# NeptuneHub/AudioMuse-AI

Hardware: NVIDIA H100
Metric: tracks_per_sec_analysed_10s_48khz (higher is better)
Workload: dtype bf16

## Files before the change

### audiomuse-ai_b200/csrc/fused_block.cu

```cuda
#include "fused_block.cuh"

#include <type_traits>

#include "gemm_wgmma.cuh"
#include "tma_pipeline.cuh"

namespace am {
namespace fused {

using namespace ptx;

constexpr int kTile = 8;
constexpr int kChunk = 64;
constexpr int kMaxCout = 256;
constexpr int kMaxStages = 4;
constexpr size_t kSmemMax = 232448;
constexpr uint32_t kConsumerBar = 1;
constexpr int kParamRows = 9 + 1 + 1;
constexpr uint32_t kDwBytes = kParamRows * kChunk * 4;
using Ring = pipe::Ring<kMaxStages>;

__host__ __device__ constexpr int halo(int S) { return (kTile - 1) * S + 3; }
__host__ __device__ constexpr int halo_px(int S) { return halo(S) * halo(S); }
__host__ __device__ constexpr int halo_rows(int S) { return (halo_px(S) + 63) / 64 * 64; }

constexpr uint32_t round1k(uint32_t v) { return (v + 1023u) & ~1023u; }

__device__ __forceinline__ int e_off(int p, int g) { return p * 64 + ((g ^ (p & 7)) << 3); }

__device__ __forceinline__ uint32_t sw128(uint32_t row, uint32_t chunk) {
  return (row << 7) + (((chunk ^ row) & 7u) << 4);
}

struct Layout {
  uint32_t stage, w2, dw;
  uint32_t xs, a2, e, bars, extra;
  int stages;
  size_t smem;
};

static Layout layout(int S, bool has_expand, int cin_p, int cout_p, int stages) {
  const uint32_t hr = (uint32_t)halo_rows(S), hpx = (uint32_t)halo_px(S);
  const uint32_t kbx = has_expand ? (uint32_t)((cin_p + 63) / 64) : 0u;
  const uint32_t n2 = (uint32_t)((cout_p + 63) / 64 * 64);
  Layout l;
  l.w2 = has_expand ? kbx * kChunk * 128 : round1k(hpx * 128);
  l.dw = l.w2 + n2 * 128;
  l.stage = round1k(l.dw + kDwBytes);
  l.xs = 0;
  l.a2 = l.xs + kbx * hr * 128;
  l.e = l.a2 + kTile * kTile * 128;
  l.bars = l.e + (has_expand ? hpx * 128 : 0u);
  l.extra = l.bars + 2 * sizeof(uint64_t);
  l.stages = stages;
  l.smem = Ring::smem_bytes(l.stage, stages, l.extra);
  return l;
}

struct Args {
  const __nv_bfloat16* X;
  const float* params;
  const float* b2;
  __nv_bfloat16* Y;
  int H, W, Ho, Wo, tiles_y, tiles_x, num_tiles;
  int cin_p, cmid_p, cout_p, residual;
  Layout l;
};

enum Phase { kRingWait, kHaloWait, kExpandMma, kExpandEpi, kDepthwise, kProjectMma, kBarrier, kEpilogue, kIssue, kNumPhases };
#ifdef AM_FUSED_PHASES
static const char* const kPhaseNames[kNumPhases] = {"ring_wait", "halo_wait", "expand_mma", "expand_epi", "depthwise",
                                                     "project_mma", "barrier", "epilogue", "issue"};
__device__ unsigned long long g_phase_cycles[3][kNumPhases];
__device__ __forceinline__ long long clock_now() {
  long long v;
  asm volatile("mov.u64 %0, %%clock64;" : "=l"(v));
  return v;
}
struct PhaseClock {
  uint32_t acc[kNumPhases];
  long long t;
  __device__ __forceinline__ PhaseClock() : acc{}, t(clock_now()) {}
  __device__ __forceinline__ void lap(Phase p) {
    const long long n = clock_now();
    acc[p] += (uint32_t)(n - t);
    t = n;
  }
  __device__ __forceinline__ void flush(int wg) {
    for (int p = 0; p < kNumPhases; ++p) atomicAdd(&g_phase_cycles[wg][p], (unsigned long long)acc[p]);
  }
};
#else
struct PhaseClock {
  __device__ __forceinline__ void lap(Phase) {}
  __device__ __forceinline__ void flush(int) {}
};
#endif

template <int S, bool kExpand>
__global__ void __launch_bounds__(pipe::kThreads, 1)
fused_block_kernel(const __grid_constant__ CUtensorMap map_x, const __grid_constant__ CUtensorMap map_w1,
                   const __grid_constant__ CUtensorMap map_w2, const Args a) {
  extern __shared__ __align__(1024) uint8_t smem_raw[];
  constexpr int HALO = halo(S), HPX = halo_px(S), HR = halo_rows(S);
  Ring ring(smem_raw, a.l.stage, a.l.stages, a.l.extra);
  uint8_t* own = ring.extra();
  uint8_t* xs = own + a.l.xs;
  uint8_t* a2 = own + a.l.a2;
  uint64_t* xs_full = reinterpret_cast<uint64_t*>(own + a.l.bars);
  uint64_t* xs_empty = xs_full + 1;

  const int per_img = a.tiles_y * a.tiles_x;
  const int kbx = (a.cin_p + 63) / 64;
  const int n2_blocks = (a.cout_p + 63) / 64;

  if (threadIdx.x == 0) {
    prefetch_tensormap(&map_x);
    if (kExpand) prefetch_tensormap(&map_w1);
    prefetch_tensormap(&map_w2);
    mbar_init(xs_full, 1);
    mbar_init(xs_empty, pipe::kConsumerThreads);
    ring.init();
  }
  __syncthreads();

  if (threadIdx.x < 128) {
    regs_producer();
    if (threadIdx.x < 32 && elect_one_sync()) {
      PhaseClock clk;
      uint32_t xs_phase = 0;
      for (int tile = blockIdx.x; tile < a.num_tiles; tile += gridDim.x) {
        const int b = tile / per_img, ty = (tile % per_img) / a.tiles_x, tx = tile % a.tiles_x;
        const int gy0 = ty * kTile * S - 1, gx0 = tx * kTile * S - 1;
        if (kExpand) {
          clk.lap(kIssue);
          mbar_wait(xs_empty, xs_phase ^ 1);
          clk.lap(kHaloWait);
          mbar_expect_tx(xs_full, (uint32_t)(kbx * HPX * 128));
          for (int kb = 0; kb < kbx; ++kb) tma_load_4d(xs + kb * HR * 128, &map_x, xs_full, kb * 64, gx0, gy0, b);
          xs_phase ^= 1;
        }
        for (int c0 = 0; c0 < a.cmid_p; c0 += kChunk) {
          const uint32_t tx_bytes = (kExpand ? (uint32_t)kbx * kChunk * 128 : (uint32_t)HPX * 128) +
                                    (uint32_t)n2_blocks * 64 * 128 + kDwBytes;
          clk.lap(kIssue);
          const Ring::Slot s = ring.acquire(tx_bytes);
          clk.lap(kRingWait);
          if (kExpand) {
            for (int kb = 0; kb < kbx; ++kb) tma_load_2d(s.smem + kb * kChunk * 128, &map_w1, s.bar, kb * 64, c0);
          } else {
            tma_load_4d(s.smem, &map_x, s.bar, c0, gx0, gy0, b);
          }
          tma_load_2d(s.smem + a.l.w2, &map_w2, s.bar, c0, 0);
          bulk_load(s.smem + a.l.dw, a.params + (int64_t)c0 * kParamRows, kDwBytes, s.bar);
        }
      }
      clk.lap(kIssue);
      clk.flush(0);
    }
    return;
  }
  regs_consumer();
  const int ct = threadIdx.x - 128;
  const int wg = __shfl_sync(0xffffffffu, ct >> 7, 0), wt = ct & 127;
  const int warp = wt >> 5, lane = wt & 31, quad = lane & 3;
  __nv_bfloat16* e_own = reinterpret_cast<__nv_bfloat16*>(own + a.l.e);
  const int nchunks = (a.cmid_p + kChunk - 1) / kChunk;
  const bool ahead = a.l.stages > 1;

  constexpr int kEN0 = ((HPX + 7) / 8 + 1) / 2 * 8;
  constexpr int kEN1 = (HPX + 7) / 8 * 8 - kEN0;
  const int half = a.cout_p / 2;

  float acc1[kEN0 / 2];
  float acc2[kMaxCout / 4];
#pragma unroll
  for (int i = 0; i < kEN0 / 2; ++i) acc1[i] = 0.f;
#pragma unroll
  for (int i = 0; i < kMaxCout / 4; ++i) acc2[i] = 0.f;

  auto expand_issue = [&](const uint8_t* stage) {
    const uint32_t w1 = smem_u32(stage), px = smem_u32(xs) + (uint32_t)(wg * kEN0 * 128);
    auto issue = [&](auto width) {
      for (int kb = 0; kb < kbx; ++kb) {
        const uint64_t da = make_smem_desc(w1 + (uint32_t)(kb * kChunk * 128));
        const uint64_t db = make_smem_desc(px + (uint32_t)(kb * HR * 128));
        const int ksteps = min(4, (a.cin_p - kb * 64) / 16);
        for (int ks = 0; ks < ksteps; ++ks)
          wgmma_into<decltype(width)::value>(acc1, da + (uint64_t)(ks * 2), db + (uint64_t)(ks * 2),
                                             (kb | ks) ? 1u : 0u);
      }
    };
    wgmma_fence();
    if (wg == 0) issue(std::integral_constant<int, kEN0>{});
    else issue(std::integral_constant<int, kEN1>{});
    wgmma_commit();
  };
  auto inside_mask = [&](int gy0, int gx0) {
    int p0 = wg * kEN0 + 2 * quad;
    asm volatile("" : "+r"(p0));
    uint64_t m = 0;
#pragma unroll
    for (int j = 0; j < kEN0 / 8; ++j)
#pragma unroll
      for (int k = 0; k < 2; ++k) {
        const int p = p0 + 8 * j + k;
        const int gy = gy0 + p / HALO, gx = gx0 + p % HALO;
        if (gy >= 0 && gy < a.H && gx >= 0 && gx < a.W) m |= 1ull << (2 * j + k);
      }
    return m;
  };
  auto expand_epilogue = [&](const uint8_t* stage, int nch, uint64_t inside) {
    reg_fence(acc1);
    const float* b1 = reinterpret_cast<const float*>(stage + a.l.dw) + 10 * kChunk;
    const int r = 16 * warp + (lane >> 2);
    const float bias[2] = {b1[r], b1[r + 8]};
    const uint32_t keep[2] = {r < nch ? ~0u : 0u, r + 8 < nch ? ~0u : 0u};
    auto pack = [&](int j, int h) {
      const uint32_t bits = (uint32_t)(inside >> (2 * j));
      const uint32_t mask = ((bits & 1u) * 0xffffu | (bits & 2u) * 0x7fff8000u) & keep[h];
      const __nv_bfloat162 v = __floats2bfloat162_rn(relu6f(acc1[4 * j + 2 * h] + bias[h]),
                                                     relu6f(acc1[4 * j + 2 * h + 1] + bias[h]));
      return *reinterpret_cast<const uint32_t*>(&v) & mask;
    };
    auto store = [&](auto wgc) {
      constexpr int P0 = decltype(wgc)::value * kEN0;
      constexpr int NG = (decltype(wgc)::value ? kEN1 : kEN0) / 8;
      constexpr int NFULL = (HPX - P0) / 8 < NG ? (HPX - P0) / 8 : NG;
      const int mi = lane >> 3;
      const uint32_t e_base = smem_u32(e_own);
#pragma unroll
      for (int j = 0; j + 1 < NFULL; j += 2) {
        const int p = P0 + 8 * (j + (mi >> 1)) + (lane & 7);
        stmatrix_x4_trans(e_base + 2 * e_off(p, 2 * warp + (mi & 1)), pack(j, 0), pack(j, 1), pack(j + 1, 0),
                          pack(j + 1, 1));
      }
      if (NFULL % 2) {
        const int p = P0 + 8 * (NFULL - 1) + (lane & 7);
        stmatrix_x2_trans(e_base + 2 * e_off(p, 2 * warp + (mi & 1)), pack(NFULL - 1, 0), pack(NFULL - 1, 1));
      }
#pragma unroll
      for (int j = NFULL; j < NG; ++j)
#pragma unroll
        for (int h = 0; h < 2; ++h) {
          const uint32_t v = pack(j, h);
#pragma unroll
          for (int k = 0; k < 2; ++k) {
            const int p = P0 + 8 * j + 2 * quad + k;
            if (p < HPX)
              reinterpret_cast<uint16_t*>(e_own)[e_off(p, 2 * warp + h) + (lane >> 2)] = (uint16_t)(v >> (16 * k));
          }
        }
    };
    if (wg == 0) store(std::integral_constant<int, 0>{});
    else store(std::integral_constant<int, 1>{});
  };

  PhaseClock clk;
  uint32_t xs_phase = 0;
  for (int tile = blockIdx.x; tile < a.num_tiles; tile += gridDim.x) {
    const int b = tile / per_img, ty = (tile % per_img) / a.tiles_x, tx = tile % a.tiles_x;
    const int oy0 = ty * kTile, ox0 = tx * kTile;
    const int gy0 = oy0 * S - 1, gx0 = ox0 * S - 1;
    const uint64_t inside = kExpand ? inside_mask(gy0, gx0) : 0;
    if (kExpand) {
      mbar_wait(xs_full, xs_phase);
      xs_phase ^= 1;
      clk.lap(kHaloWait);
      const uint8_t* s0 = ring.wait_ptr();
      clk.lap(kRingWait);
      expand_issue(s0);
      wgmma_wait<0>();
      clk.lap(kExpandMma);
      expand_epilogue(s0, min(kChunk, a.cmid_p), inside);
      if (nchunks == 1) mbar_arrive(xs_empty);
      clk.lap(kExpandEpi);
    }

    for (int c = 0; c < nchunks; ++c) {
      const int c0 = c * kChunk, nch = min(kChunk, a.cmid_p - c0);
      const bool next = kExpand && c + 1 < nchunks;
      uint8_t* sp = ring.wait_ptr();
      clk.lap(kRingWait);
      const float* dwp = reinterpret_cast<const float*>(sp + a.l.dw);
      const __nv_bfloat16* e = kExpand ? e_own : reinterpret_cast<const __nv_bfloat16*>(sp);
      named_bar_sync(kConsumerBar, pipe::kConsumerThreads);
      clk.lap(kBarrier);
      const uint8_t* sn = nullptr;
      if (next && ahead) {
        sn = ring.wait_ahead_ptr();
        clk.lap(kRingWait);
        expand_issue(sn);
        clk.lap(kExpandMma);
      }

      {
        const int ox = ct >> 5, cp = lane, g = cp >> 2;
        uint32_t out[kTile] = {};
        if (2 * cp < nch) {
          float2 w[9];
#pragma unroll
          for (int t = 0; t < 9; ++t) w[t] = *reinterpret_cast<const float2*>(dwp + t * kChunk + 2 * cp);
          const float2 bias = *reinterpret_cast<const float2*>(dwp + 9 * kChunk + 2 * cp);
          float2 acc[kTile];
#pragma unroll
          for (int oy = 0; oy < kTile; ++oy) acc[oy] = bias;
          const __nv_bfloat16* col[8];
#pragma unroll
          for (int k = 0; k < 8; ++k) col[k] = e + ox * S * 64 + ((g ^ ((ox * S + k) & 7)) << 3) + 2 * (cp & 3);
#pragma unroll
          for (int iy = 0; iy < HALO; ++iy) {
            float2 v[3];
#pragma unroll
            for (int dx = 0; dx < 3; ++dx) {
              const int d = iy * HALO + dx;
              v[dx] = __bfloat1622float2(*reinterpret_cast<const __nv_bfloat162*>(col[d & 7] + d * 64));
            }
#pragma unroll
            for (int dy = 0; dy < 3; ++dy) {
              if (iy < dy || (iy - dy) % S != 0 || (iy - dy) / S >= kTile) continue;
              const int oy = (iy - dy) / S;
#pragma unroll
              for (int dx = 0; dx < 3; ++dx) {
                acc[oy].x = fmaf(v[dx].x, w[dy * 3 + dx].x, acc[oy].x);
                acc[oy].y = fmaf(v[dx].y, w[dy * 3 + dx].y, acc[oy].y);
              }
            }
          }
#pragma unroll
          for (int oy = 0; oy < kTile; ++oy) {
            const __nv_bfloat162 o = __floats2bfloat162_rn(relu6f(acc[oy].x), relu6f(acc[oy].y));
            out[oy] = *reinterpret_cast<const uint32_t*>(&o);
          }
        }
        uint8_t* arow = a2 + sw128(ox, g) + 4 * (cp & 3);
#pragma unroll
        for (int oy = 0; oy < kTile; ++oy) *reinterpret_cast<uint32_t*>(arow + oy * kTile * 128) = out[oy];
      }
      fence_proxy_async();
      clk.lap(kDepthwise);
      named_bar_sync(kConsumerBar, pipe::kConsumerThreads);
      clk.lap(kBarrier);

      wgmma_fence();
      {
        const uint64_t da = make_smem_desc(smem_u32(a2));
        const uint64_t db = make_smem_desc(smem_u32(sp) + a.l.w2 + (uint32_t)(wg * half * 128));
        auto project = [&](auto width) {
          for (int ks = 0; ks < nch / 16; ++ks)
            wgmma_into<decltype(width)::value>(acc2, da + (uint64_t)(ks * 2), db + (uint64_t)(ks * 2),
                                               (c0 | ks) ? 1u : 0u);
        };
        switch (half) {
          case 8: project(std::integral_constant<int, 8>{}); break;
          case 16: project(std::integral_constant<int, 16>{}); break;
          case 24: project(std::integral_constant<int, 24>{}); break;
          case 32: project(std::integral_constant<int, 32>{}); break;
          case 40: project(std::integral_constant<int, 40>{}); break;
          case 48: project(std::integral_constant<int, 48>{}); break;
          case 56: project(std::integral_constant<int, 56>{}); break;
          case 64: project(std::integral_constant<int, 64>{}); break;
          case 72: project(std::integral_constant<int, 72>{}); break;
          case 80: project(std::integral_constant<int, 80>{}); break;
          case 88: project(std::integral_constant<int, 88>{}); break;
          case 96: project(std::integral_constant<int, 96>{}); break;
          case 104: project(std::integral_constant<int, 104>{}); break;
          case 112: project(std::integral_constant<int, 112>{}); break;
          case 120: project(std::integral_constant<int, 120>{}); break;
          case 128: project(std::integral_constant<int, 128>{}); break;
        }
      }
      wgmma_commit();
      clk.lap(kProjectMma);

      if (next && !ahead) {
        wgmma_wait<0>();
        ring.release();
        sn = ring.wait_ptr();
        clk.lap(kRingWait);
        expand_issue(sn);
      }
      wgmma_wait<0>();
      reg_fence(acc2);
      if (!next || ahead) ring.release();
      clk.lap(kProjectMma);
      if (next) {
        expand_epilogue(sn, min(kChunk, a.cmid_p - c0 - kChunk), inside);
        if (c + 2 == nchunks) mbar_arrive(xs_empty);
        clk.lap(kExpandEpi);
      }
    }

#pragma unroll
    for (int h = 0; h < 2; ++h) {
      const int px = warp * 16 + (lane >> 2) + 8 * h;
      const int oy = oy0 + (px >> 3), ox = ox0 + (px & 7);
      if (oy >= a.Ho || ox >= a.Wo) continue;
      const int64_t pix = ((int64_t)b * a.Ho + oy) * a.Wo + ox;
#pragma unroll
      for (int j = 0; j < kMaxCout / 16; ++j) {
        if (8 * j >= half) break;
        const int n = wg * half + 8 * j + 2 * quad;
        float f0 = acc2[4 * j + 2 * h] + __ldg(&a.b2[n]);
        float f1 = acc2[4 * j + 2 * h + 1] + __ldg(&a.b2[n + 1]);
        if (a.residual) {
          const float2 r = __bfloat1622float2(*reinterpret_cast<const __nv_bfloat162*>(a.X + pix * a.cin_p + n));
          f0 += r.x;
          f1 += r.y;
        }
        *reinterpret_cast<__nv_bfloat162*>(a.Y + pix * a.cout_p + n) = __floats2bfloat162_rn(f0, f1);
      }
    }
    clk.lap(kEpilogue);
  }
  if (wt == 0) clk.flush(1 + wg);
}

static bool fits(const BlockDesc& d) {
  const size_t hr = (size_t)halo_rows(d.stride);
  const size_t kbx = d.has_expand ? (size_t)((d.cin_p + 63) / 64) : 0;
  const size_t n2 = (size_t)((d.cout_p + 63) / 64 * 64);
  const size_t set = kbx * hr * 128 + kbx * kChunk * 128 + n2 * 128 + 64 * 128 + hr * 128;
  return set + 1024 <= kSmemMax;
}

bool plan(const BlockDesc& d, Plan* out) {
  if (d.stride != 1 && d.stride != 2) return false;
  if (d.cout_p > kMaxCout || d.cout_p % 16 || d.cmid_p % 16 || d.cin_p % 16) return false;
  if (!d.has_expand && d.cin_p != d.cmid_p) return false;
  if (d.residual && (d.stride != 1 || d.cin_p != d.cout_p)) return false;
  if (!fits(d)) return false;
  Layout l = layout(d.stride, d.has_expand != 0, d.cin_p, d.cout_p, kMaxStages);
  for (int s = kMaxStages - 1; s >= 1 && l.smem > kSmemMax; --s) l = layout(d.stride, d.has_expand != 0, d.cin_p, d.cout_p, s);
  out->stages = l.stages;
  out->smem_bytes = l.smem;
  return out->smem_bytes <= kSmemMax;
}

template <int S, bool kExpand>
static int launch(const CUtensorMap& mx, const CUtensorMap& m1, const CUtensorMap& m2, const Args& a, size_t smem,
                  cudaStream_t st) {
  AM_TRY((allow_dynamic_smem<fused_block_kernel<S, kExpand>>(kSmemMax)));
  const int grid = std::max(1, std::min(a.num_tiles, sm_count()));
#ifdef AM_FUSED_PHASES
  void* counters = nullptr;
  AM_CUDA(cudaGetSymbolAddress(&counters, g_phase_cycles));
  AM_CUDA(cudaMemsetAsync(counters, 0, sizeof(g_phase_cycles), st));
#endif
  AM_LAUNCH((fused_block_kernel<S, kExpand>), grid, pipe::kThreads, smem, st, mx, m1, m2, a);
#ifdef AM_FUSED_PHASES
  unsigned long long c[3][kNumPhases];
  AM_CUDA(cudaStreamSynchronize(st));
  AM_CUDA(cudaMemcpyFromSymbol(c, g_phase_cycles, sizeof(c)));
  std::fprintf(stderr, "fused_phases H=%d W=%d cin=%d cmid=%d cout=%d S=%d stages=%d grid=%d tiles=%d", a.H, a.W,
               a.cin_p, a.cmid_p, a.cout_p, S, a.l.stages, grid, a.num_tiles);
  for (int w = 0; w < 3; ++w)
    for (int p = 0; p < kNumPhases; ++p) std::fprintf(stderr, " wg%d.%s=%llu", w, kPhaseNames[p], c[w][p]);
  std::fprintf(stderr, "\n");
#endif
  return AM_OK;
}

std::vector<float> pack_params(const std::vector<float>& wd, const std::vector<float>& bd, const std::vector<float>* b1,
                               int c_p) {
  const int chunks = (c_p + kChunk - 1) / kChunk;
  std::vector<float> out((size_t)chunks * kParamRows * kChunk, 0.f);
  for (int c = 0; c < c_p; ++c) {
    float* q = &out[((size_t)(c / kChunk) * kParamRows) * kChunk + c % kChunk];
    for (int t = 0; t < 9; ++t) q[t * kChunk] = wd[(size_t)t * c_p + c];
    q[9 * kChunk] = bd[c];
    if (b1) q[10 * kChunk] = (*b1)[c];
  }
  return out;
}

int run(const BlockDesc& d, const Plan& p, const __nv_bfloat16* X, const __nv_bfloat16* W1, const float* params,
        const __nv_bfloat16* W2, const float* b2, __nv_bfloat16* Y, int B, cudaStream_t st) {
  AM_CHECK(X && params && W2 && b2 && Y && (!d.has_expand || W1), "fused block: NULL operand");
  auto aligned16 = [](const void* q) { return (reinterpret_cast<uintptr_t>(q) & 15) == 0; };
  AM_CHECK(aligned16(X) && aligned16(W2) && aligned16(params) && (!d.has_expand || aligned16(W1)),
           "fused block: operands must be 16-byte aligned (TMA)");
  Args a{};
  a.X = X;
  a.params = params;
  a.b2 = b2;
  a.Y = Y;
  a.H = d.H;
  a.W = d.W;
  a.Ho = (d.H - 1) / d.stride + 1;
  a.Wo = (d.W - 1) / d.stride + 1;
  a.tiles_y = (a.Ho + kTile - 1) / kTile;
  a.tiles_x = (a.Wo + kTile - 1) / kTile;
  const int64_t tiles = (int64_t)B * a.tiles_y * a.tiles_x;
  AM_CHECK(tiles < ((int64_t)1 << 31), "fused block: %lld tiles is too many for one launch", (long long)tiles);
  a.num_tiles = (int)tiles;
  a.cin_p = d.cin_p;
  a.cmid_p = d.cmid_p;
  a.cout_p = d.cout_p;
  a.residual = d.residual;
  const Layout l = layout(d.stride, d.has_expand != 0, d.cin_p, d.cout_p, p.stages);
  AM_CHECK(l.smem == p.smem_bytes, "fused block: plan does not match the block");
  a.l = l;

  CUtensorMap mx, m1, m2;
  const int hl = halo(d.stride);
  AM_TRY(gemm::encode_map_nhwc_bf16(&mx, X, B, d.H, d.W, d.cin_p, hl, hl, true));
  AM_TRY(gemm::encode_map_bf16(&m2, W2, d.cmid_p, d.cout_p, d.cmid_p, (d.cout_p + 63) / 64 * 64));
  if (d.has_expand) AM_TRY(gemm::encode_map_bf16(&m1, W1, d.cin_p, d.cmid_p, d.cin_p, kChunk));
  else m1 = m2;
  if (d.stride == 1) return d.has_expand ? launch<1, true>(mx, m1, m2, a, l.smem, st) : launch<1, false>(mx, m1, m2, a, l.smem, st);
  return d.has_expand ? launch<2, true>(mx, m1, m2, a, l.smem, st) : launch<2, false>(mx, m1, m2, a, l.smem, st);
}

}
}
```

### audiomuse-ai_b200/csrc/fused_block.cuh

```cuda
#pragma once

#include "common.cuh"

namespace am {
namespace fused {

struct BlockDesc {
  int H, W;
  int cin_p, cmid_p, cout_p;
  int stride;
  int has_expand;
  int residual;
};

struct Plan {
  size_t smem_bytes = 0;
  int stages = 1;
};

bool plan(const BlockDesc& d, Plan* out);

std::vector<float> pack_params(const std::vector<float>& wd, const std::vector<float>& bd, const std::vector<float>* b1,
                               int c_p);

int run(const BlockDesc& d, const Plan& p, const __nv_bfloat16* X, const __nv_bfloat16* W1, const float* params,
        const __nv_bfloat16* W2, const float* b2, __nv_bfloat16* Y, int B, cudaStream_t st);

}
}
```

### audiomuse-ai_b200/csrc/gemm.cu

```cuda
#include "gemm_wgmma.cuh"
#include "tma_pipeline.cuh"

#include <mutex>

namespace am {
namespace gemm {

using pipe::kChunkK;
using pipe::kThreads;

constexpr int kBlockM = 128;
constexpr int kStages = 4;
constexpr int kATileBytes = kBlockM * kChunkK * 2;
constexpr int kMaxBlockN = 256;
constexpr size_t kSmemMax = 232448;
using Ring = pipe::Ring<kStages>;

using namespace ptx;

struct KernelArgs {
  int64_t M, N;
  int K;
  int block_n;
  int tiles_m, tiles_n;
// ... 196 lines not shown
  }
  if (!args.d_is_f32 && wt == 0) bulk_wait_group<0>();
}

__global__ void gemm_simt_kernel(const __nv_bfloat16* __restrict__ A, int64_t M, int64_t lda,
                                 const __nv_bfloat16* __restrict__ B, int64_t N, int64_t ldb, int K,
                                 KernelArgs args) {
  const int64_t n = (int64_t)blockIdx.x * blockDim.x + threadIdx.x;
  const int64_t m = blockIdx.y;
  if (n >= N || m >= M) return;
  float acc = 0.f;
  for (int k = 0; k < K; ++k) acc = fmaf(__bfloat162float(A[m * lda + k]), __bfloat162float(B[n * ldb + k]), acc);
  float v = acc * args.alpha;
  if (args.bias) v += args.bias[n];
  if (args.col_sub) v -= args.col_sub[n];
  if (args.act == 1) v = relu6f(v);
  else if (args.act == 2) v = fmaxf(v, 0.f);
  else if (args.act == 3) v *= fminf(fmaxf(fmaf(v, 1.0f / 6.0f, 0.5f), 0.f), 1.f);
  if (args.d_is_f32) {
    reinterpret_cast<float*>(args.D)[m * args.ldd + n] = v;
  } else {
    if (args.residual) v += __bfloat162float(args.residual[m * args.ld_res + n]);
    reinterpret_cast<__nv_bfloat16*>(args.D)[m * args.ldd + n] = __float2bfloat16_rn(v);
  }
}

typedef CUresult (*EncodeTiledFn)(CUtensorMap*, CUtensorMapDataType, cuuint32_t, void*, const cuuint64_t*,
                                  const cuuint64_t*, const cuuint32_t*, const cuuint32_t*, CUtensorMapInterleave,
                                  CUtensorMapSwizzle, CUtensorMapL2promotion, CUtensorMapFloatOOBfill);

static EncodeTiledFn g_encode = nullptr;
static std::once_flag g_encode_once;

static EncodeTiledFn get_encode() {
  std::call_once(g_encode_once, [] {
    void* fn = nullptr;
    cudaDriverEntryPointQueryResult qres;
    cudaError_t e = cudaGetDriverEntryPoint("cuTensorMapEncodeTiled", &fn, cudaEnableDefault, &qres);
    if (e == cudaSuccess && qres == cudaDriverEntryPointSuccess) g_encode = reinterpret_cast<EncodeTiledFn>(fn);
    cudaGetLastError();
  });
  return g_encode;
}

bool available() { return ensure_init() == AM_OK && device_cc() == 90 && get_encode() != nullptr; }

int encode_map_bf16(void* map_out, const void* base, int64_t inner, int64_t rows, int64_t pitch_elems, int box_rows) {
  AM_CHECK(get_encode() != nullptr, "cuTensorMapEncodeTiled unavailable");
  const cuuint64_t dims[2] = {(cuuint64_t)inner, (cuuint64_t)rows};
  const cuuint64_t strides[1] = {(cuuint64_t)pitch_elems * 2};
  const cuuint32_t box[2] = {(cuuint32_t)kChunkK, (cuuint32_t)box_rows};
  const cuuint32_t estr[2] = {1, 1};
  CUresult r = get_encode()(reinterpret_cast<CUtensorMap*>(map_out), CU_TENSOR_MAP_DATA_TYPE_BFLOAT16, 2,
                            const_cast<void*>(base), dims, strides, box, estr, CU_TENSOR_MAP_INTERLEAVE_NONE,
                            CU_TENSOR_MAP_SWIZZLE_128B, CU_TENSOR_MAP_L2_PROMOTION_L2_256B,
                            CU_TENSOR_MAP_FLOAT_OOB_FILL_NONE);
  if (r != CUDA_SUCCESS) {
    set_error("cuTensorMapEncodeTiled failed (%d) inner=%lld rows=%lld pitch=%lld box_rows=%d", (int)r,
              (long long)inner, (long long)rows, (long long)pitch_elems, box_rows);
    return AM_ERR_CUDA;
  }
  return AM_OK;
}

int encode_map_nhwc_bf16(void* map_out, const void* base, int64_t n, int64_t h, int64_t w, int64_t c, int box_w,
                         int box_h, bool swizzle) {
  AM_CHECK(get_encode() != nullptr, "cuTensorMapEncodeTiled unavailable");
  const cuuint64_t dims[4] = {(cuuint64_t)c, (cuuint64_t)w, (cuuint64_t)h, (cuuint64_t)n};
  const cuuint64_t strides[3] = {(cuuint64_t)(c * 2), (cuuint64_t)(w * c * 2), (cuuint64_t)(h * w * c * 2)};
  const cuuint32_t box[4] = {(cuuint32_t)kChunkK, (cuuint32_t)box_w, (cuuint32_t)box_h, 1};
  const cuuint32_t estr[4] = {1, 1, 1, 1};
  CUresult r = get_encode()(reinterpret_cast<CUtensorMap*>(map_out), CU_TENSOR_MAP_DATA_TYPE_BFLOAT16, 4,
                            const_cast<void*>(base), dims, strides, box, estr, CU_TENSOR_MAP_INTERLEAVE_NONE,
                            swizzle ? CU_TENSOR_MAP_SWIZZLE_128B : CU_TENSOR_MAP_SWIZZLE_NONE,
                            CU_TENSOR_MAP_L2_PROMOTION_L2_256B, CU_TENSOR_MAP_FLOAT_OOB_FILL_NONE);
  if (r != CUDA_SUCCESS) {
    set_error("cuTensorMapEncodeTiled failed (%d) nhwc=[%lld, %lld, %lld, %lld] box=%dx%d", (int)r, (long long)n,
              (long long)h, (long long)w, (long long)c, box_w, box_h);
    return AM_ERR_CUDA;
  }
  return AM_OK;
}

static int encode_map_d(CUtensorMap* map_out, void* D, int64_t cols, int64_t rows, int64_t pitch_elems, int box_cols) {
  const cuuint64_t dims[2] = {(cuuint64_t)cols, (cuuint64_t)rows};
  const cuuint64_t strides[1] = {(cuuint64_t)pitch_elems * 2};
  const cuuint32_t box[2] = {(cuuint32_t)box_cols, 64};
  const cuuint32_t estr[2] = {1, 1};
  const int sw = box_cols == 64 ? 128 : tail_swizzle_bytes(box_cols);
  const CUtensorMapSwizzle swizzle = sw == 128  ? CU_TENSOR_MAP_SWIZZLE_128B
                                     : sw == 64 ? CU_TENSOR_MAP_SWIZZLE_64B
                                     : sw == 32 ? CU_TENSOR_MAP_SWIZZLE_32B
                                                : CU_TENSOR_MAP_SWIZZLE_NONE;
  CUresult r = get_encode()(map_out, CU_TENSOR_MAP_DATA_TYPE_BFLOAT16, 2, D, dims, strides, box, estr,
                            CU_TENSOR_MAP_INTERLEAVE_NONE, swizzle, CU_TENSOR_MAP_L2_PROMOTION_NONE,
                            CU_TENSOR_MAP_FLOAT_OOB_FILL_NONE);
  if (r != CUDA_SUCCESS) {
    set_error("cuTensorMapEncodeTiled failed (%d) for D: cols=%lld rows=%lld pitch=%lld box_cols=%d", (int)r,
              (long long)cols, (long long)rows, (long long)pitch_elems, box_cols);
    return AM_ERR_CUDA;
  }
  return AM_OK;
}

static bool gemm_has_n(int n) {
  return n == 16 || n == 32 || n == 48 || n == 64 || n == 80 || n == 96 || n == 112 || n == 128 || n == 144 ||
         n == 160 || n == 192 || n == 224 || n == 256;
}

static int tile_n_for(int n) {
  for (int c = 16; c <= kMaxBlockN; c += 16)
    if (c >= n && gemm_has_n(c)) return c;
  return kMaxBlockN;
}

static int pick_block_n(int64_t N, bool chunk_max) {
  const int64_t n16 = (int64_t)round_up((size_t)N, 16);
  int bn;
  if (n16 <= kMaxBlockN) {
    bn = (int)n16;
  } else if (!chunk_max) {
    int best = kMaxBlockN;
    for (int c = kMaxBlockN; c >= 128; c -= 16) {
      if (!gemm_has_n(c)) continue;
      if ((N + c - 1) / c * c < (N + best - 1) / best * best) best = c;
    }
    return best;
  } else {
    const int64_t tiles = (n16 + kMaxBlockN - 1) / kMaxBlockN;
    bn = (int)round_up((size_t)((n16 + tiles - 1) / tiles), 16);
  }
  if (chunk_max) bn = std::min(kMaxBlockN, (int)round_up((size_t)bn, 32));
  return tile_n_for(bn);
}

static KernelArgs make_args(int64_t M, int64_t N, int K, void* D, int64_t ldd, bool d_is_f32, const Epilogue& ep,
                            bool m_fastest) {
  KernelArgs a{};
  a.M = M;
  a.N = N;
  a.K = K;
  a.block_n = pick_block_n(N, ep.chunk_max != nullptr);
  a.tiles_m = (int)((M + kBlockM - 1) / kBlockM);
  a.tiles_n = (int)((N + a.block_n - 1) / a.block_n);
  a.m_fastest = m_fastest ? 1 : 0;
  a.D = D;
  a.ldd = ldd;
  a.d_is_f32 = d_is_f32 ? 1 : 0;
  a.d_vec = (ldd % 2 == 0 && (reinterpret_cast<uintptr_t>(D) & (d_is_f32 ? 7 : 3)) == 0) ? 1 : 0;
  a.alpha = ep.alpha;
  a.bias = ep.bias;
  a.col_sub = ep.col_sub;
  a.act = ep.act;
  a.chunk_max = ep.chunk_max;
  a.ld_cm = ep.ld_cm;
  a.residual = ep.residual;
  a.ld_res = ep.ld_res;
  return a;
}

template <int BN>
static int launch_bn(const CUtensorMap& map_a, const CUtensorMap& map_b, KernelArgs& args, cudaStream_t st) {
  AM_TRY(allow_dynamic_smem<gemm_wgmma_kernel<BN>>(kSmemMax));
  CUtensorMap map_d = map_a, map_d_tail = map_a;
  if (!args.d_is_f32) {
    if (BN >= 64) AM_TRY(encode_map_d(&map_d, args.D, args.N, args.M, args.ldd, 64));
    if (BN % 64 != 0) AM_TRY(encode_map_d(&map_d_tail, args.D, args.N, args.M, args.ldd, BN % 64));
  }
  const size_t stage_bytes = (size_t)kATileBytes + (size_t)BN * kChunkK * 2;
  const size_t extra = args.d_is_f32 ? 0 : 2 * (size_t)gemm::stage_bytes<BN>();
  args.stages = (int)std::min<size_t>(kStages, (kSmemMax - Ring::smem_bytes(0, 0, extra)) / stage_bytes);
  const size_t smem = Ring::smem_bytes(stage_bytes, args.stages, extra);
  const int tiles = args.tiles_m * args.tiles_n;
  const int grid = std::max(1, std::min(tiles, sm_count()));
  AM_LAUNCH(gemm_wgmma_kernel<BN>, grid, kThreads, smem, st, map_a, map_b, map_d, map_d_tail, args);
  return AM_OK;
}

int gemm_bf16(const __nv_bfloat16* A, int64_t M, int64_t lda, const __nv_bfloat16* B, int64_t N, int64_t ldb, int K,
              void* D, int64_t ldd, bool d_is_f32, const Epilogue& ep, bool m_fastest, cudaStream_t st) {
  AM_CHECK(A && B && D, "gemm: NULL operand");
  AM_CHECK(M > 0 && N > 0 && K > 0, "gemm: empty problem M=%lld N=%lld K=%d", (long long)M, (long long)N, K);
// ... 45 lines not shown
```

### audiomuse-ai_b200/csrc/gemm_wgmma.cuh

```cuda
#pragma once

#include "common.cuh"

namespace am {
namespace gemm {

struct Epilogue {
  float alpha = 1.0f;
  const float* bias = nullptr;
  const float* col_sub = nullptr;
  int act = 0;
  const __nv_bfloat16* residual = nullptr;
  int64_t ld_res = 0;
  float* chunk_max = nullptr;
  int64_t ld_cm = 0;
};

bool available();

int gemm_bf16(const __nv_bfloat16* A, int64_t M, int64_t lda, const __nv_bfloat16* B, int64_t N,
              int64_t ldb, int K, void* D, int64_t ldd, bool d_is_f32, const Epilogue& ep,
              bool m_fastest, cudaStream_t st);

int encode_map_bf16(void* map_out, const void* base, int64_t inner, int64_t rows, int64_t pitch_elems, int box_rows);

int encode_map_nhwc_bf16(void* map_out, const void* base, int64_t n, int64_t h, int64_t w, int64_t c, int box_w,
                         int box_h, bool swizzle);

int gemm_bf16_simt(const __nv_bfloat16* A, int64_t M, int64_t lda, const __nv_bfloat16* B, int64_t N,
                   int64_t ldb, int K, void* D, int64_t ldd, bool d_is_f32, const Epilogue& ep,
                   cudaStream_t st);

inline int scores_bf16(const __nv_bfloat16* Qb, int qrows, const __nv_bfloat16* Xb, int64_t N, int dpad, float* S,
                       int64_t ldS, float* CM, int64_t ldCM, const float* xnorm2, cudaStream_t st) {
  Epilogue ep;
  ep.alpha = xnorm2 ? 2.0f : 1.0f;
  ep.col_sub = xnorm2;
  ep.chunk_max = CM;
  ep.ld_cm = CM ? ldCM : 0;
  return gemm_bf16(Qb, qrows, dpad, Xb, N, dpad, dpad, S, ldS, true, ep, true, st);
}

}
}
```

### audiomuse-ai_b200/csrc/ptx_sm90.cuh

```cuda
#pragma once

#include <cuda.h>

#include "common.cuh"

namespace am {
namespace ptx {

__device__ __forceinline__ uint32_t smem_u32(const void* p) {
  return static_cast<uint32_t>(__cvta_generic_to_shared(p));
}
__device__ __forceinline__ bool elect_one_sync() {
  uint32_t pred;
  asm volatile(
      "{\n"
      ".reg .pred P;\n"
      "elect.sync _|P, 0xffffffff;\n"
      "selp.b32 %0, 1, 0, P;\n"
      "}\n"
      : "=r"(pred));
  return pred != 0;
}
__device__ __forceinline__ void mbar_init(uint64_t* bar, uint32_t count) {
  asm volatile("mbarrier.init.shared::cta.b64 [%0], %1;" ::"r"(smem_u32(bar)), "r"(count));
}
__device__ __forceinline__ void mbar_expect_tx(uint64_t* bar, uint32_t bytes) {
  asm volatile("mbarrier.arrive.expect_tx.shared::cta.b64 _, [%0], %1;" ::"r"(smem_u32(bar)), "r"(bytes)
               : "memory");
}
__device__ __forceinline__ void mbar_arrive(uint64_t* bar) {
  asm volatile("mbarrier.arrive.shared::cta.b64 _, [%0];" ::"r"(smem_u32(bar)) : "memory");
}
__device__ __forceinline__ void mbar_wait(uint64_t* bar, uint32_t parity) {
  asm volatile(
      "{\n"
      ".reg .pred P1;\n"
      "LAB_WAIT:\n"
      "mbarrier.try_wait.parity.shared::cta.b64 P1, [%0], %1;\n"
      "@P1 bra DONE;\n"
      "bra LAB_WAIT;\n"
      "DONE:\n"
      "}\n" ::"r"(smem_u32(bar)),
      "r"(parity)
      : "memory");
}
__device__ __forceinline__ void fence_barrier_init() {
  asm volatile("fence.mbarrier_init.release.cluster;" ::: "memory");
}
__device__ __forceinline__ void fence_proxy_async() {
  asm volatile("fence.proxy.async.shared::cta;" ::: "memory");
}
__device__ __forceinline__ void tma_load_2d(void* smem_dst, const CUtensorMap* map, uint64_t* bar, int c0,
                                            int c1) {
  asm volatile(
      "cp.async.bulk.tensor.2d.shared::cluster.global.mbarrier::complete_tx::bytes [%0], [%1, {%3, %4}], [%2];"
      ::"r"(smem_u32(smem_dst)),
      "l"(reinterpret_cast<uint64_t>(map)), "r"(smem_u32(bar)), "r"(c0), "r"(c1)
      : "memory");
}
__device__ __forceinline__ void tma_load_4d(void* smem_dst, const CUtensorMap* map, uint64_t* bar, int c0, int c1,
                                            int c2, int c3) {
  asm volatile(
      "cp.async.bulk.tensor.4d.shared::cluster.global.mbarrier::complete_tx::bytes [%0], [%1, {%3, %4, %5, %6}], [%2];"
      ::"r"(smem_u32(smem_dst)),
      "l"(reinterpret_cast<uint64_t>(map)), "r"(smem_u32(bar)), "r"(c0), "r"(c1), "r"(c2), "r"(c3)
      : "memory");
}
__device__ __forceinline__ void bulk_load(void* smem_dst, const void* src, uint32_t bytes, uint64_t* bar) {
  asm volatile(
      "cp.async.bulk.shared::cluster.global.mbarrier::complete_tx::bytes [%0], [%1], %2, [%3];"
      ::"r"(smem_u32(smem_dst)), "l"(reinterpret_cast<uint64_t>(src)), "r"(bytes), "r"(smem_u32(bar))
      : "memory");
}
__device__ __forceinline__ void tma_store_2d(const CUtensorMap* map, const void* smem_src, int c0, int c1) {
  asm volatile("cp.async.bulk.tensor.2d.global.shared::cta.bulk_group [%0, {%2, %3}], [%1];"
               ::"l"(reinterpret_cast<uint64_t>(map)), "r"(smem_u32(smem_src)), "r"(c0), "r"(c1)
               : "memory");
}
__device__ __forceinline__ void bulk_commit_group() { asm volatile("cp.async.bulk.commit_group;" ::: "memory"); }
template <int N>
__device__ __forceinline__ void bulk_wait_group_read() {
  asm volatile("cp.async.bulk.wait_group.read %0;" ::"n"(N) : "memory");
}
template <int N>
__device__ __forceinline__ void bulk_wait_group() {
  asm volatile("cp.async.bulk.wait_group %0;" ::"n"(N) : "memory");
}
__device__ __forceinline__ void named_bar_sync(uint32_t id, uint32_t count) {
  asm volatile("bar.sync %0, %1;" ::"r"(id), "r"(count) : "memory");
}
__device__ __forceinline__ void prefetch_tensormap(const CUtensorMap* map) {
  asm volatile("prefetch.tensormap [%0];" ::"l"(reinterpret_cast<uint64_t>(map)) : "memory");
}

__device__ __forceinline__ void regs_producer() { asm volatile("setmaxnreg.dec.sync.aligned.u32 40;" ::: "memory"); }
__device__ __forceinline__ void regs_consumer() { asm volatile("setmaxnreg.inc.sync.aligned.u32 232;" ::: "memory"); }

__device__ __forceinline__ void wgmma_fence() { asm volatile("wgmma.fence.sync.aligned;" ::: "memory"); }
__device__ __forceinline__ void wgmma_commit() { asm volatile("wgmma.commit_group.sync.aligned;" ::: "memory"); }
__device__ __forceinline__ void wgmma_wait_all() { asm volatile("wgmma.wait_group.sync.aligned 0;" ::: "memory"); }
template <int N>
__device__ __forceinline__ void wgmma_wait() { asm volatile("wgmma.wait_group.sync.aligned %0;" ::"n"(N) : "memory"); }
template <int R>
__device__ __forceinline__ void reg_fence(float (&d)[R]) {
#pragma unroll
  for (int i = 0; i < R; ++i) asm volatile("" : "+f"(d[i])::"memory");
}

__device__ __forceinline__ uint64_t make_smem_desc(uint32_t smem_addr) {
  uint64_t d = 0;
  d |= (uint64_t)((smem_addr >> 4) & 0x3fffu);
  d |= (uint64_t)1 << 16;
  d |= (uint64_t)(1024u >> 4) << 32;
  d |= (uint64_t)1 << 62;
  return d;
}

template <int N>
struct Wgmma;
template <>
struct Wgmma<8> {
  __device__ __forceinline__ static void mma(float (&d)[4], uint64_t desc_a, uint64_t desc_b, uint32_t scale_d) {
    asm volatile(
        "{\n.reg .pred p;\nsetp.ne.b32 p, %6, 0;\n"
        "wgmma.mma_async.sync.aligned.m64n8k16.f32.bf16.bf16 {%0, %1, %2, %3}, %4, %5, p, 1, 1, 0, 0;\n}\n"
        : "+f"(d[0]), "+f"(d[1]), "+f"(d[2]), "+f"(d[3])
        : "l"(desc_a), "l"(desc_b), "r"(scale_d));
  }
};
template <>
struct Wgmma<16> {
  __device__ __forceinline__ static void mma(float (&d)[8], uint64_t desc_a, uint64_t desc_b, uint32_t scale_d) {
    asm volatile(
        "{\n.reg .pred p;\nsetp.ne.b32 p, %10, 0;\n"
        "wgmma.mma_async.sync.aligned.m64n16k16.f32.bf16.bf16 {%0, %1, %2, %3, %4, %5, %6, %7}, %8, %9, p, 1, 1, 0, 0;\n}\n"
        : "+f"(d[0]), "+f"(d[1]), "+f"(d[2]), "+f"(d[3]), "+f"(d[4]), "+f"(d[5]), "+f"(d[6]), "+f"(d[7])
        : "l"(desc_a), "l"(desc_b), "r"(scale_d));
  }
};
template <>
struct Wgmma<24> {
  __device__ __forceinline__ static void mma(float (&d)[12], uint64_t desc_a, uint64_t desc_b, uint32_t scale_d) {
    asm volatile(
        "{\n.reg .pred p;\nsetp.ne.b32 p, %14, 0;\n"
        "wgmma.mma_async.sync.aligned.m64n24k16.f32.bf16.bf16 {%0, %1, %2, %3, %4, %5, %6, %7, %8, %9, %10, %11}, %12, %13, p, 1, 1, 0, 0;\n}\n"
        : "+f"(d[0]), "+f"(d[1]), "+f"(d[2]), "+f"(d[3]), "+f"(d[4]), "+f"(d[5]), "+f"(d[6]), "+f"(d[7]), "+f"(d[8]), "+f"(d[9]), "+f"(d[10]), "+f"(d[11])
        : "l"(desc_a), "l"(desc_b), "r"(scale_d));
  }
};
template <>
struct Wgmma<32> {
  __device__ __forceinline__ static void mma(float (&d)[16], uint64_t desc_a, uint64_t desc_b, uint32_t scale_d) {
    asm volatile(
        "{\n.reg .pred p;\nsetp.ne.b32 p, %18, 0;\n"
        "wgmma.mma_async.sync.aligned.m64n32k16.f32.bf16.bf16 {%0, %1, %2, %3, %4, %5, %6, %7, %8, %9, %10, %11, %12, %13, %14, %15}, %16, %17, p, 1, 1, 0, 0;\n}\n"
        : "+f"(d[0]), "+f"(d[1]), "+f"(d[2]), "+f"(d[3]), "+f"(d[4]), "+f"(d[5]), "+f"(d[6]), "+f"(d[7]), "+f"(d[8]), "+f"(d[9]), "+f"(d[10]), "+f"(d[11]), "+f"(d[12]), "+f"(d[13]), "+f"(d[14]), "+f"(d[15])
        : "l"(desc_a), "l"(desc_b), "r"(scale_d));
  }
};
template <>
struct Wgmma<40> {
// ... 197 lines not shown
```

Baseline: 10880.

## Stage fused block output in shared memory and write via TMA stores

```diff
diff --git a/audiomuse-ai_b200/csrc/fused_block.cu b/audiomuse-ai_b200/csrc/fused_block.cu
--- a/audiomuse-ai_b200/csrc/fused_block.cu
+++ b/audiomuse-ai_b200/csrc/fused_block.cu
@@ -34,25 +34,29 @@
 
 struct Layout {
   uint32_t stage, w2, dw;
-  uint32_t xs, a2, e, bars, extra;
+  uint32_t xs, a2, e, stg, b2, bars, extra;
   int stages;
+  int staged;
   size_t smem;
 };
 
-static Layout layout(int S, bool has_expand, int cin_p, int cout_p, int stages) {
+static Layout layout(int S, bool has_expand, int cin_p, int cout_p, int stages, bool staged, int w2_rows) {
   const uint32_t hr = (uint32_t)halo_rows(S), hpx = (uint32_t)halo_px(S);
   const uint32_t kbx = has_expand ? (uint32_t)((cin_p + 63) / 64) : 0u;
-  const uint32_t n2 = (uint32_t)((cout_p + 63) / 64 * 64);
   Layout l;
   l.w2 = has_expand ? kbx * kChunk * 128 : round1k(hpx * 128);
-  l.dw = l.w2 + n2 * 128;
+  l.dw = l.w2 + (uint32_t)w2_rows * 128;
   l.stage = round1k(l.dw + kDwBytes);
   l.xs = 0;
   l.a2 = l.xs + kbx * hr * 128;
   l.e = l.a2 + kTile * kTile * 128;
-  l.bars = l.e + (has_expand ? hpx * 128 : 0u);
+  const uint32_t e_end = l.e + (has_expand ? hpx * 128 : 0u);
+  l.stg = staged ? round1k(e_end) : e_end;
+  l.b2 = l.stg + (staged ? kTile * kTile * (uint32_t)cout_p * 2 : 0u);
+  l.bars = l.b2 + (uint32_t)cout_p * 4;
   l.extra = l.bars + 2 * sizeof(uint64_t);
   l.stages = stages;
+  l.staged = staged ? 1 : 0;
   l.smem = Ring::smem_bytes(l.stage, stages, l.extra);
   return l;
 }
@@ -97,10 +101,20 @@
 };
 #endif
 
+__device__ __forceinline__ uint32_t stg_off(int r, int c, int cout_p) {
+  const int full = cout_p & ~(kChunk - 1);
+  if (c < full) return (uint32_t)((c >> 6) * 8192 + r * 128 + (c & 7) * 2) + ((((uint32_t)(c >> 3) ^ (uint32_t)r) & 7u) << 4);
+  const int tail = cout_p - full;
+  const uint32_t o = (uint32_t)(r * tail * 2 + (c - full) * 2);
+  const uint32_t sw = tail == 16 ? ((o >> 7) & 1u) << 4 : tail == 32 ? ((o >> 7) & 3u) << 4 : 0u;
+  return (uint32_t)full * 128u + (o ^ sw);
+}
+
 template <int S, bool kExpand>
 __global__ void __launch_bounds__(pipe::kThreads, 1)
 fused_block_kernel(const __grid_constant__ CUtensorMap map_x, const __grid_constant__ CUtensorMap map_w1,
-                   const __grid_constant__ CUtensorMap map_w2, const Args a) {
+                   const __grid_constant__ CUtensorMap map_w2, const __grid_constant__ CUtensorMap map_y,
+                   const __grid_constant__ CUtensorMap map_y_tail, const Args a) {
   extern __shared__ __align__(1024) uint8_t smem_raw[];
   constexpr int HALO = halo(S), HPX = halo_px(S), HR = halo_rows(S);
   Ring ring(smem_raw, a.l.stage, a.l.stages, a.l.extra);
@@ -112,12 +126,14 @@
 
   const int per_img = a.tiles_y * a.tiles_x;
   const int kbx = (a.cin_p + 63) / 64;
-  const int n2_blocks = (a.cout_p + 63) / 64;
+  const bool staged = kExpand && a.l.staged;
 
   if (threadIdx.x == 0) {
     prefetch_tensormap(&map_x);
     if (kExpand) prefetch_tensormap(&map_w1);
     prefetch_tensormap(&map_w2);
+    if (staged && a.cout_p >= kChunk) prefetch_tensormap(&map_y);
+    if (staged && a.cout_p % kChunk) prefetch_tensormap(&map_y_tail);
     mbar_init(xs_full, 1);
     mbar_init(xs_empty, pipe::kConsumerThreads);
     ring.init();
@@ -142,7 +158,7 @@
         }
         for (int c0 = 0; c0 < a.cmid_p; c0 += kChunk) {
           const uint32_t tx_bytes = (kExpand ? (uint32_t)kbx * kChunk * 128 : (uint32_t)HPX * 128) +
-                                    (uint32_t)n2_blocks * 64 * 128 + kDwBytes;
+                                    (uint32_t)a.cout_p * 128 + kDwBytes;
           clk.lap(kIssue);
           const Ring::Slot s = ring.acquire(tx_bytes);
           clk.lap(kRingWait);
@@ -167,6 +183,10 @@
   __nv_bfloat16* e_own = reinterpret_cast<__nv_bfloat16*>(own + a.l.e);
   const int nchunks = (a.cmid_p + kChunk - 1) / kChunk;
   const bool ahead = a.l.stages > 1;
+  const bool res = S == 1 && a.residual;
+  uint8_t* stg = own + a.l.stg;
+  float* b2s = reinterpret_cast<float*>(own + a.l.b2);
+  for (int i = ct; i < a.cout_p; i += pipe::kConsumerThreads) b2s[i] = a.b2[i];
 
   constexpr int kEN0 = ((HPX + 7) / 8 + 1) / 2 * 8;
   constexpr int kEN1 = (HPX + 7) / 8 * 8 - kEN0;
@@ -256,6 +276,16 @@
     else store(std::integral_constant<int, 1>{});
   };
 
+  auto stage_residual = [&](const uint8_t* blk, int kb) {
+    const int ng = min(kChunk, a.cout_p - kb * kChunk) / 8;
+    for (int i = ct; i < kTile * kTile * ng; i += pipe::kConsumerThreads) {
+      const int q = i / ng, g = i - q * ng;
+      const int p = ((q >> 3) + 1) * HALO + (q & 7) + 1;
+      *reinterpret_cast<uint4*>(stg + stg_off(q, kb * kChunk + 8 * g, a.cout_p)) =
+          *reinterpret_cast<const uint4*>(blk + sw128((uint32_t)p, (uint32_t)g));
+    }
+  };
+
   PhaseClock clk;
   uint32_t xs_phase = 0;
   for (int tile = blockIdx.x; tile < a.num_tiles; tile += gridDim.x) {
@@ -273,7 +303,6 @@
       wgmma_wait<0>();
       clk.lap(kExpandMma);
       expand_epilogue(s0, min(kChunk, a.cmid_p), inside);
-      if (nchunks == 1) mbar_arrive(xs_empty);
       clk.lap(kExpandEpi);
     }
 
@@ -284,6 +313,7 @@
       clk.lap(kRingWait);
       const float* dwp = reinterpret_cast<const float*>(sp + a.l.dw);
       const __nv_bfloat16* e = kExpand ? e_own : reinterpret_cast<const __nv_bfloat16*>(sp);
+      if (staged && ct == 0 && c == (res ? 0 : nchunks - 1)) bulk_wait_group_read<0>();
       named_bar_sync(kConsumerBar, pipe::kConsumerThreads);
       clk.lap(kBarrier);
       const uint8_t* sn = nullptr;
@@ -293,6 +323,11 @@
         expand_issue(sn);
         clk.lap(kExpandMma);
       }
+      if (staged && res && c == 0) {
+        for (int kb = 0; kb < kbx; ++kb) stage_residual(xs + kb * HR * 128, kb);
+        clk.lap(kEpilogue);
+      }
+      if (kExpand && nchunks == 1) mbar_arrive(xs_empty);
 
       {
         const int ox = ct >> 5, cp = lane, g = cp >> 2;
@@ -391,28 +426,52 @@
       }
     }
 
+    int px0 = warp * 16 + (lane >> 2), n0 = wg * half + 2 * quad;
+    asm volatile("" : "+r"(px0), "+r"(n0));
 #pragma unroll
     for (int h = 0; h < 2; ++h) {
-      const int px = warp * 16 + (lane >> 2) + 8 * h;
+      const int px = px0 + 8 * h;
       const int oy = oy0 + (px >> 3), ox = ox0 + (px & 7);
-      if (oy >= a.Ho || ox >= a.Wo) continue;
+      const bool direct = !staged && oy < a.Ho && ox < a.Wo;
       const int64_t pix = ((int64_t)b * a.Ho + oy) * a.Wo + ox;
 #pragma unroll
       for (int j = 0; j < kMaxCout / 16; ++j) {
         if (8 * j >= half) break;
-        const int n = wg * half + 8 * j + 2 * quad;
-        float f0 = acc2[4 * j + 2 * h] + __ldg(&a.b2[n]);
-        float f1 = acc2[4 * j + 2 * h + 1] + __ldg(&a.b2[n + 1]);
-        if (a.residual) {
-          const float2 r = __bfloat1622float2(*reinterpret_cast<const __nv_bfloat162*>(a.X + pix * a.cin_p + n));
-          f0 += r.x;
-          f1 += r.y;
+        const int n = n0 + 8 * j;
+        const float2 bias = *reinterpret_cast<const float2*>(b2s + n);
+        float f0 = acc2[4 * j + 2 * h] + bias.x;
+        float f1 = acc2[4 * j + 2 * h + 1] + bias.y;
+        if (staged) {
+          __nv_bfloat162* q = reinterpret_cast<__nv_bfloat162*>(stg + stg_off(px, n, a.cout_p));
+          if (res) {
+            const float2 r = __bfloat1622float2(*q);
+            f0 += r.x;
+            f1 += r.y;
+          }
+          *q = __floats2bfloat162_rn(f0, f1);
+        } else if (direct) {
+          if (res) {
+            const float2 r = __bfloat1622float2(*reinterpret_cast<const __nv_bfloat162*>(a.X + pix * a.cin_p + n));
+            f0 += r.x;
+            f1 += r.y;
+          }
+          *reinterpret_cast<__nv_bfloat162*>(a.Y + pix * a.cout_p + n) = __floats2bfloat162_rn(f0, f1);
         }
-        *reinterpret_cast<__nv_bfloat162*>(a.Y + pix * a.cout_p + n) = __floats2bfloat162_rn(f0, f1);
+      }
+    }
+    if (staged) {
+      fence_proxy_async();
+      named_bar_sync(kConsumerBar, pipe::kConsumerThreads);
+      if (ct == 0) {
+        const int full = a.cout_p & ~(kChunk - 1);
+        for (int c0 = 0; c0 < full; c0 += kChunk) tma_store_4d(&map_y, stg + c0 * 128, c0, ox0, oy0, b);
+        if (full < a.cout_p) tma_store_4d(&map_y_tail, stg + full * 128, full, ox0, oy0, b);
+        bulk_commit_group();
       }
     }
     clk.lap(kEpilogue);
   }
+  if (staged && ct == 0) bulk_wait_group<0>();
   if (wt == 0) clk.flush(1 + wg);
 }
 
@@ -430,16 +489,21 @@
   if (!d.has_expand && d.cin_p != d.cmid_p) return false;
   if (d.residual && (d.stride != 1 || d.cin_p != d.cout_p)) return false;
   if (!fits(d)) return false;
-  Layout l = layout(d.stride, d.has_expand != 0, d.cin_p, d.cout_p, kMaxStages);
-  for (int s = kMaxStages - 1; s >= 1 && l.smem > kSmemMax; --s) l = layout(d.stride, d.has_expand != 0, d.cin_p, d.cout_p, s);
+  const bool ex = d.has_expand != 0;
+  Layout l = layout(d.stride, ex, d.cin_p, d.cout_p, kMaxStages, false, (d.cout_p + 63) / 64 * 64);
+  for (int s = kMaxStages - 1; s >= 1 && l.smem > kSmemMax; --s)
+    l = layout(d.stride, ex, d.cin_p, d.cout_p, s, false, (d.cout_p + 63) / 64 * 64);
+  const Layout staged = layout(d.stride, ex, d.cin_p, d.cout_p, l.stages, true, d.cout_p);
+  l = ex && staged.smem <= kSmemMax ? staged : layout(d.stride, ex, d.cin_p, d.cout_p, l.stages, false, d.cout_p);
   out->stages = l.stages;
+  out->staged = l.staged;
   out->smem_bytes = l.smem;
   return out->smem_bytes <= kSmemMax;
 }
 
 template <int S, bool kExpand>
-static int launch(const CUtensorMap& mx, const CUtensorMap& m1, const CUtensorMap& m2, const Args& a, size_t smem,
-                  cudaStream_t st) {
+static int launch(const CUtensorMap& mx, const CUtensorMap& m1, const CUtensorMap& m2, const CUtensorMap& my,
+                  const CUtensorMap& my_tail, const Args& a, size_t smem, cudaStream_t st) {
   AM_TRY((allow_dynamic_smem<fused_block_kernel<S, kExpand>>(kSmemMax)));
   const int grid = std::max(1, std::min(a.num_tiles, sm_count()));
 #ifdef AM_FUSED_PHASES
@@ -447,13 +511,13 @@
   AM_CUDA(cudaGetSymbolAddress(&counters, g_phase_cycles));
   AM_CUDA(cudaMemsetAsync(counters, 0, sizeof(g_phase_cycles), st));
 #endif
-  AM_LAUNCH((fused_block_kernel<S, kExpand>), grid, pipe::kThreads, smem, st, mx, m1, m2, a);
+  AM_LAUNCH((fused_block_kernel<S, kExpand>), grid, pipe::kThreads, smem, st, mx, m1, m2, my, my_tail, a);
 #ifdef AM_FUSED_PHASES
   unsigned long long c[3][kNumPhases];
   AM_CUDA(cudaStreamSynchronize(st));
   AM_CUDA(cudaMemcpyFromSymbol(c, g_phase_cycles, sizeof(c)));
-  std::fprintf(stderr, "fused_phases H=%d W=%d cin=%d cmid=%d cout=%d S=%d stages=%d grid=%d tiles=%d", a.H, a.W,
-               a.cin_p, a.cmid_p, a.cout_p, S, a.l.stages, grid, a.num_tiles);
+  std::fprintf(stderr, "fused_phases H=%d W=%d cin=%d cmid=%d cout=%d S=%d stages=%d grid=%d tiles=%d staged=%d", a.H,
+               a.W, a.cin_p, a.cmid_p, a.cout_p, S, a.l.stages, grid, a.num_tiles, a.l.staged);
   for (int w = 0; w < 3; ++w)
     for (int p = 0; p < kNumPhases; ++p) std::fprintf(stderr, " wg%d.%s=%llu", w, kPhaseNames[p], c[w][p]);
   std::fprintf(stderr, "\n");
@@ -498,19 +562,28 @@
   a.cmid_p = d.cmid_p;
   a.cout_p = d.cout_p;
   a.residual = d.residual;
-  const Layout l = layout(d.stride, d.has_expand != 0, d.cin_p, d.cout_p, p.stages);
+  const Layout l = layout(d.stride, d.has_expand != 0, d.cin_p, d.cout_p, p.stages, p.staged != 0, d.cout_p);
   AM_CHECK(l.smem == p.smem_bytes, "fused block: plan does not match the block");
+  AM_CHECK(!l.staged || aligned16(Y), "fused block: the output must be 16-byte aligned (TMA stores)");
   a.l = l;
 
-  CUtensorMap mx, m1, m2;
+  CUtensorMap mx, m1, m2, my, my_tail;
   const int hl = halo(d.stride);
   AM_TRY(gemm::encode_map_nhwc_bf16(&mx, X, B, d.H, d.W, d.cin_p, hl, hl, true));
-  AM_TRY(gemm::encode_map_bf16(&m2, W2, d.cmid_p, d.cout_p, d.cmid_p, (d.cout_p + 63) / 64 * 64));
+  AM_TRY(gemm::encode_map_bf16(&m2, W2, d.cmid_p, d.cout_p, d.cmid_p, d.cout_p));
   if (d.has_expand) AM_TRY(gemm::encode_map_bf16(&m1, W1, d.cin_p, d.cmid_p, d.cin_p, kChunk));
   else m1 = m2;
-  if (d.stride == 1) return d.has_expand ? launch<1, true>(mx, m1, m2, a, l.smem, st) : launch<1, false>(mx, m1, m2, a, l.smem, st);
-  return d.has_expand ? launch<2, true>(mx, m1, m2, a, l.smem, st) : launch<2, false>(mx, m1, m2, a, l.smem, st);
-}
-
-}
-}
+  my = my_tail = mx;
+  const int tail = d.cout_p % kChunk;
+  if (l.staged && d.cout_p >= kChunk)
+    AM_TRY(gemm::encode_map_nhwc_store_bf16(&my, Y, B, a.Ho, a.Wo, d.cout_p, kChunk, kTile, kTile));
+  if (l.staged && tail) AM_TRY(gemm::encode_map_nhwc_store_bf16(&my_tail, Y, B, a.Ho, a.Wo, d.cout_p, tail, kTile, kTile));
+  if (d.stride == 1)
+    return d.has_expand ? launch<1, true>(mx, m1, m2, my, my_tail, a, l.smem, st)
+                        : launch<1, false>(mx, m1, m2, my, my_tail, a, l.smem, st);
+  return d.has_expand ? launch<2, true>(mx, m1, m2, my, my_tail, a, l.smem, st)
+                      : launch<2, false>(mx, m1, m2, my, my_tail, a, l.smem, st);
+}
+
+}
+}
diff --git a/audiomuse-ai_b200/csrc/fused_block.cuh b/audiomuse-ai_b200/csrc/fused_block.cuh
--- a/audiomuse-ai_b200/csrc/fused_block.cuh
+++ b/audiomuse-ai_b200/csrc/fused_block.cuh
@@ -16,6 +16,7 @@
 struct Plan {
   size_t smem_bytes = 0;
   int stages = 1;
+  int staged = 0;
 };
 
 bool plan(const BlockDesc& d, Plan* out);
diff --git a/audiomuse-ai_b200/csrc/gemm.cu b/audiomuse-ai_b200/csrc/gemm.cu
--- a/audiomuse-ai_b200/csrc/gemm.cu
+++ b/audiomuse-ai_b200/csrc/gemm.cu
@@ -302,22 +302,44 @@
   return AM_OK;
 }
 
+static CUtensorMapSwizzle store_swizzle(int box_cols) {
+  const int sw = box_cols == 64 ? 128 : tail_swizzle_bytes(box_cols);
+  return sw == 128  ? CU_TENSOR_MAP_SWIZZLE_128B
+         : sw == 64 ? CU_TENSOR_MAP_SWIZZLE_64B
+         : sw == 32 ? CU_TENSOR_MAP_SWIZZLE_32B
+                    : CU_TENSOR_MAP_SWIZZLE_NONE;
+}
+
 static int encode_map_d(CUtensorMap* map_out, void* D, int64_t cols, int64_t rows, int64_t pitch_elems, int box_cols) {
   const cuuint64_t dims[2] = {(cuuint64_t)cols, (cuuint64_t)rows};
   const cuuint64_t strides[1] = {(cuuint64_t)pitch_elems * 2};
   const cuuint32_t box[2] = {(cuuint32_t)box_cols, 64};
   const cuuint32_t estr[2] = {1, 1};
-  const int sw = box_cols == 64 ? 128 : tail_swizzle_bytes(box_cols);
-  const CUtensorMapSwizzle swizzle = sw == 128  ? CU_TENSOR_MAP_SWIZZLE_128B
-                                     : sw == 64 ? CU_TENSOR_MAP_SWIZZLE_64B
-                                     : sw == 32 ? CU_TENSOR_MAP_SWIZZLE_32B
-                                                : CU_TENSOR_MAP_SWIZZLE_NONE;
   CUresult r = get_encode()(map_out, CU_TENSOR_MAP_DATA_TYPE_BFLOAT16, 2, D, dims, strides, box, estr,
-                            CU_TENSOR_MAP_INTERLEAVE_NONE, swizzle, CU_TENSOR_MAP_L2_PROMOTION_NONE,
+                            CU_TENSOR_MAP_INTERLEAVE_NONE, store_swizzle(box_cols), CU_TENSOR_MAP_L2_PROMOTION_NONE,
                             CU_TENSOR_MAP_FLOAT_OOB_FILL_NONE);
   if (r != CUDA_SUCCESS) {
     set_error("cuTensorMapEncodeTiled failed (%d) for D: cols=%lld rows=%lld pitch=%lld box_cols=%d", (int)r,
               (long long)cols, (long long)rows, (long long)pitch_elems, box_cols);
+    return AM_ERR_CUDA;
+  }
+  return AM_OK;
+}
+
+int encode_map_nhwc_store_bf16(void* map_out, void* base, int64_t n, int64_t h, int64_t w, int64_t c, int box_c,
+                               int box_w, int box_h) {
+  AM_CHECK(get_encode() != nullptr, "cuTensorMapEncodeTiled unavailable");
+  AM_CHECK(box_c == 16 || box_c == 32 || box_c == 48 || box_c == 64, "NHWC store map: box of %d channels", box_c);
+  const cuuint64_t dims[4] = {(cuuint64_t)c, (cuuint64_t)w, (cuuint64_t)h, (cuuint64_t)n};
+  const cuuint64_t strides[3] = {(cuuint64_t)(c * 2), (cuuint64_t)(w * c * 2), (cuuint64_t)(h * w * c * 2)};
+  const cuuint32_t box[4] = {(cuuint32_t)box_c, (cuuint32_t)box_w, (cuuint32_t)box_h, 1};
+  const cuuint32_t estr[4] = {1, 1, 1, 1};
+  CUresult r = get_encode()(reinterpret_cast<CUtensorMap*>(map_out), CU_TENSOR_MAP_DATA_TYPE_BFLOAT16, 4, base, dims,
+                            strides, box, estr, CU_TENSOR_MAP_INTERLEAVE_NONE, store_swizzle(box_c),
+                            CU_TENSOR_MAP_L2_PROMOTION_NONE, CU_TENSOR_MAP_FLOAT_OOB_FILL_NONE);
+  if (r != CUDA_SUCCESS) {
+    set_error("cuTensorMapEncodeTiled failed (%d) for an NHWC store: [%lld, %lld, %lld, %lld] box=%dx%dx%d", (int)r,
+              (long long)n, (long long)h, (long long)w, (long long)c, box_c, box_w, box_h);
     return AM_ERR_CUDA;
   }
   return AM_OK;
diff --git a/audiomuse-ai_b200/csrc/gemm_wgmma.cuh b/audiomuse-ai_b200/csrc/gemm_wgmma.cuh
--- a/audiomuse-ai_b200/csrc/gemm_wgmma.cuh
+++ b/audiomuse-ai_b200/csrc/gemm_wgmma.cuh
@@ -27,6 +27,9 @@
 int encode_map_nhwc_bf16(void* map_out, const void* base, int64_t n, int64_t h, int64_t w, int64_t c, int box_w,
                          int box_h, bool swizzle);
 
+int encode_map_nhwc_store_bf16(void* map_out, void* base, int64_t n, int64_t h, int64_t w, int64_t c, int box_c,
+                               int box_w, int box_h);
+
 int gemm_bf16_simt(const __nv_bfloat16* A, int64_t M, int64_t lda, const __nv_bfloat16* B, int64_t N,
                    int64_t ldb, int K, void* D, int64_t ldd, bool d_is_f32, const Epilogue& ep,
                    cudaStream_t st);
diff --git a/audiomuse-ai_b200/csrc/ptx_sm90.cuh b/audiomuse-ai_b200/csrc/ptx_sm90.cuh
--- a/audiomuse-ai_b200/csrc/ptx_sm90.cuh
+++ b/audiomuse-ai_b200/csrc/ptx_sm90.cuh
@@ -77,6 +77,12 @@
                ::"l"(reinterpret_cast<uint64_t>(map)), "r"(smem_u32(smem_src)), "r"(c0), "r"(c1)
                : "memory");
 }
+__device__ __forceinline__ void tma_store_4d(const CUtensorMap* map, const void* smem_src, int c0, int c1, int c2,
+                                             int c3) {
+  asm volatile("cp.async.bulk.tensor.4d.global.shared::cta.bulk_group [%0, {%2, %3, %4, %5}], [%1];"
+               ::"l"(reinterpret_cast<uint64_t>(map)), "r"(smem_u32(smem_src)), "r"(c0), "r"(c1), "r"(c2), "r"(c3)
+               : "memory");
+}
 __device__ __forceinline__ void bulk_commit_group() { asm volatile("cp.async.bulk.commit_group;" ::: "memory"); }
 template <int N>
 __device__ __forceinline__ void bulk_wait_group_read() {
```

Measured after the change: 11110, median of 6. 2.1% higher.
